# mcogoni/supersdr

Measured on AMD Instinct MI355X. Metric: real-time IQ channels sustained (WF+demod), higher is better.
Workload: dtype f32

## Files before the change

supersdr_amd/csrc/ssdr_audio_dev.h:

```cpp
#pragma once
#include "ssdr_math.h"
#include "ssdr_kernels.h"

constexpr int OCT = 10;
constexpr int NOCT = (SSDR_HIST + SSDR_FRAME) / 8;
constexpr int HOCT = SSDR_HIST / 8;
typedef uint32_t u32x4 __attribute__((ext_vector_type(4)));

SSDR_DEV void lds_sync()
{
    __builtin_amdgcn_fence(__ATOMIC_RELEASE, "wavefront");
    __builtin_amdgcn_wave_barrier();
    __builtin_amdgcn_fence(__ATOMIC_ACQUIRE, "wavefront");
}

template <int CTRL, int ROWMASK>
SSDR_DEV float dpp(float identity, float x)
{
    return __int_as_float(__builtin_amdgcn_update_dpp(__float_as_int(identity), __float_as_int(x), CTRL, ROWMASK, 0xF, false));
}
SSDR_DEV float vmax(float a, float b)
{
    float r;
    asm("v_max_f32 %0, %1, %2" : "=v"(r) : "v"(a), "v"(b));
    return r;
}
SSDR_DEV float vmax3(float a, float b, float c)
{
    float r;
    asm("v_max3_f32 %0, %1, %2, %3" : "=v"(r) : "v"(a), "v"(b), "v"(c));
    return r;
}
SSDR_DEV float vmax3_abs(float a, float b, float c)
{
    float r;
    asm("v_max3_f32 %0, %1, |%2|, |%3|" : "=v"(r) : "v"(a), "v"(b), "v"(c));
    return r;
}
SSDR_DEV uint32_t lane63_u(uint32_t x) { return (uint32_t)__builtin_amdgcn_readlane((int)x, 63); }
SSDR_DEV uint32_t from_prev_lane_u(uint32_t lane0_value, uint32_t x)
{
    return (uint32_t)__builtin_amdgcn_update_dpp((int)lane0_value, (int)x, 0x138, 0xF, 0xF, false);
}
typedef short s16x2 __attribute__((ext_vector_type(2)));
SSDR_DEV uint32_t iq_power(uint32_t raw)
{
    uint32_t p;
    asm("v_dot2_i32_i16 %0, %1, %1, 0" : "=v"(p) : "v"(raw));
    return p;
}
SSDR_DEV float lane63(float x) { return __int_as_float(__builtin_amdgcn_readlane(__float_as_int(x), 63)); }
SSDR_DEV float from_prev_lane(float lane0_value, float x) { return dpp<0x138, 0xF>(lane0_value, x); }

#define SSDR_SCAN6(STEP) STEP("row_shr:1", "0xf") STEP("row_shr:2", "0xf") STEP("row_shr:4", "0xf") STEP("row_shr:8", "0xf") \
                         STEP("row_bcast:15", "0xa") STEP("row_bcast:31", "0xc")
#define SSDR_DPP(C, M) " " C " row_mask:" M " bank_mask:0xf"

SSDR_DEV float scan_max(float x)
{
#define STEP(C, M) asm("s_nop 1\n\tv_max_f32_dpp %0, %0, %0" SSDR_DPP(C, M) : "+v"(x));
    SSDR_SCAN6(STEP)
#undef STEP
    return x;
}
SSDR_DEV float scan_sum(float x)
{
#define STEP(C, M) asm("s_nop 1\n\tv_add_f32_dpp %0, %0, %0" SSDR_DPP(C, M) : "+v"(x));
    SSDR_SCAN6(STEP)
#undef STEP
    return x;
}
SSDR_DEV void scan_affine(float &A, float &B)
{
#define STEP(C, M) asm("s_nop 1\n\tv_fmac_f32_dpp %1, %1, %0" SSDR_DPP(C, M) "\n\tv_mul_f32_dpp %0, %0, %0" SSDR_DPP(C, M) : "+v"(A), "+v"(B));
    SSDR_SCAN6(STEP)
#undef STEP
}

struct Nco {
    uint32_t dphi;
    float cs, ss;
    float qc, qs;
    float tc, ts;
};
SSDR_DEV void nco_setup(Nco &n, uint32_t dphi, int l, int block = 8)
{
    n.dphi = dphi;
    ssdr_phasor32(dphi, n.cs, n.ss);
    ssdr_phasor32((uint32_t)(block * l) * dphi, n.qc, n.qs);
    n.tc = 1.0f; n.ts = 0.0f;
}
SSDR_DEV void nco_frame_table(Nco &n, uint32_t phase_of_frame, int l, int frame = SSDR_FRAME)
{
    ssdr_phasor32(phase_of_frame + (uint32_t)(frame * l) * n.dphi, n.tc, n.ts);
}
SSDR_DEV float lane_f(float x, uint32_t lane) { return __int_as_float(__builtin_amdgcn_readlane(__float_as_int(x), (int)lane)); }
SSDR_DEV void nco_block(const Nco &n, uint32_t f, float &c, float &s)
{
    const float fc = lane_f(n.tc, f & 63u), fs = lane_f(n.ts, f & 63u);
    c = fmaf(fc, n.qc, -(fs * n.qs));
    s = fmaf(fs, n.qc, fc * n.qs);
}
SSDR_DEV void phasor_mul(float ac, float as, float bc, float bs, float &c, float &s)
{
    c = fmaf(ac, bc, -(as * bs));
    s = fmaf(as, bc, ac * bs);
}

template <bool CLIP, int N = 8>
SSDR_DEV void mix8(const uint32_t (&rw)[N], float c, float s, float cs, float ss, float2 (&z)[N], float &amax)
{
#pragma unroll
    for (int j = 0; j < N; j++) {
        const float xr = (float)(int16_t)(rw[j] & 0xFFFFu);
        const float xi = (float)((int32_t)rw[j] >> 16);
        if (CLIP) amax = vmax3_abs(amax, xr, xi);
        z[j] = make_float2(fmaf(xr, c, xi * s), fmaf(xi, c, -(xr * s)));
        const float cn = fmaf(c, cs, -(s * ss)), sn = fmaf(s, cs, c * ss);
        c = cn; s = sn;
    }
}

template <bool CLIP>
SSDR_DEV void mix8_carry(const uint32_t *rw, float &c, float &s, float cs, float ss, float2 (&z)[8], float &amax)
{
#pragma unroll
    for (int j = 0; j < 8; j++) {
        const float xr = (float)(int16_t)(rw[j] & 0xFFFFu);
        const float xi = (float)((int32_t)rw[j] >> 16);
        if (CLIP) amax = vmax3_abs(amax, xr, xi);
        z[j] = make_float2(fmaf(xr, c, xi * s), fmaf(xi, c, -(xr * s)));
        const float cn = fmaf(c, cs, -(s * ss)), sn = fmaf(s, cs, c * ss);
        c = cn; s = sn;
    }
}

SSDR_DEV void load_oct(const float2 *z, int q, float2 (&v)[8])
{
    const float4 *p = reinterpret_cast<const float4 *>(z + q * OCT);
#pragma unroll
    for (int i = 0; i < 4; i++) {
        const float4 t = p[i];
        v[2 * i] = make_float2(t.x, t.y);
        v[2 * i + 1] = make_float2(t.z, t.w);
    }
}

SSDR_DEV void store_oct(float2 *z, int q, const float2 (&v)[8])
{
    float4 *p = reinterpret_cast<float4 *>(z + q * OCT);
#pragma unroll
    for (int i = 0; i < 4; i++) p[i] = make_float4(v[2 * i].x, v[2 * i].y, v[2 * i + 1].x, v[2 * i + 1].y);
}

template <int K0, int NK>
SSDR_DEV void fir_taps(const float *h, const float2 (&A)[8], const float2 (&B)[8], float (&yr)[8], float (&yi)[8])
{
#pragma unroll
    for (int kk = K0; kk < K0 + NK; kk++) {
#pragma unroll
        for (int j = 0; j < 8; j++) {
            const float2 v = (j - kk >= 0) ? A[(j - kk) & 7] : B[(8 + j - kk) & 7];
            yr[j] = fmaf(h[kk], v.x, yr[j]);
            yi[j] = fmaf(h[kk], v.y, yi[j]);
        }
    }
}


struct AgcK { float c0, c1, knee, d8; uint32_t K; };

template <bool INTEGER_POWER>
SSDR_DEV void demod_am(const float (&p)[8], float &dc, float (&aud)[8])
{
    constexpr float DC_APOW[8] = SSDR_DC_APOW_INIT;
    float env[8], loc[8];
    float s = 0.0f;
#pragma unroll
    for (int j = 0; j < 8; j++) {
        env[j] = INTEGER_POWER ? ssdr_sqrt_rn_int(p[j]) : ssdr_sqrt_rn(p[j]);
        s = fmaf(SSDR_DC_A, s, SSDR_DC_AL * env[j]);
        loc[j] = s;
    }
    float Asc = DC_APOW[7], Bsc = s;
    scan_affine(Asc, Bsc);
    const float Ae = from_prev_lane(1.0f, Asc), Be = from_prev_lane(0.0f, Bsc);
    const float carry = fmaf(Ae, dc, Be);
    float m = 0.0f;
#pragma unroll
    for (int j = 0; j < 8; j++) {
        m = fmaf(DC_APOW[j], carry, loc[j]);
        aud[j] = env[j] - m;
    }
    dc = lane63(m);
}

SSDR_DEV void demod_ssb(const float (&yr)[8], const float (&yi)[8], float c, float s, float cs2, float ss2, float (&aud)[8])
{
#pragma unroll
    for (int j = 0; j < 8; j++) {
        aud[j] = fmaf(yr[j], c, -(yi[j] * s));
        const float cn = fmaf(c, cs2, -(s * ss2)), sn = fmaf(s, cs2, c * ss2);
        c = cn; s = sn;
    }
}

SSDR_DEV void demod_fm(const float (&yr)[8], const float (&yi)[8], float prev_re, float prev_im, float kfm, float (&aud)[8])
{
    float pr = from_prev_lane(prev_re, yr[7]), pi = from_prev_lane(prev_im, yi[7]);
#pragma unroll
    for (int j = 0; j < 8; j++) {
        const float dr = fmaf(yr[j], pr, yi[j] * pi);
        const float di = fmaf(yi[j], pr, -(yr[j] * pi));
        aud[j] = ssdr_atan2p(di, dr) * kfm;
        pr = yr[j]; pi = yi[j];
    }
}

SSDR_DEV float block_peak(const float (&p)[8])
{
    return vmax3(vmax3(vmax3(p[0], p[1], p[2]), p[3], p[4]), vmax3(p[5], p[6], p[7]), SSDR_P_FLOOR);
}

SSDR_DEV float agc_pack_store(const float (&p)[8], const float (&aud)[8], int l, const AgcK &k, float &agc_d,
                              float (&agc_m)[8], int16_t *dst, float pm_known = -1.0f)
{
    const float pm = pm_known >= 0.0f ? pm_known : block_peak(p);
    const float al = ssdr_log2p(pm);
    const float fl = (float)l;
    const float d8 = k.d8;
    float e;
    if (k.K == 0) {
        const float P = scan_max(fmaf(fl, d8, al));
        e = vmax(fmaf(-fl, d8, P), fmaf(-(fl + 1.0f), d8, agc_d));
        agc_d = lane63(e);
    } else {
        const float P = scan_max(al);
        float maxM = agc_m[0], mK = agc_m[0];
#pragma unroll
        for (int i = 1; i < 8; i++)
            if ((uint32_t)i < k.K) { maxM = fmaxf(maxM, agc_m[i]); mK = agc_m[i]; }
        e = vmax(vmax(P, maxM), fmaf(-(fl + 1.0f), d8, agc_d));
        agc_d = fmaxf(fmaf(-64.0f, d8, agc_d), mK);
#pragma unroll
        for (int i = 7; i > 0; i--) agc_m[i] = agc_m[i - 1];
        agc_m[0] = lane63(P);
    }
    const float g = ssdr_exp2p(fmaf(k.c1, vmax(e, k.knee), k.c0));
    u32x4 w;
#pragma unroll
    for (int j = 0; j < 8; j += 2) {
        const int i0 = __float2int_rn(aud[j] * g), i1 = __float2int_rn(aud[j + 1] * g);
        w[j >> 1] = __builtin_bit_cast(uint32_t, __builtin_amdgcn_cvt_pk_i16(i0, i1));
    }
    SSDR_NT_STORE(w, reinterpret_cast<u32x4 *>(dst));
    return g;
}

SSDR_DEV void iq_pack_store(const float (&yr)[8], const float (&yi)[8], float g, uint32_t *dst)
{
    u32x4 w0, w1;
#pragma unroll
    for (int j = 0; j < 8; j++) {
        const uint32_t v = __builtin_bit_cast(uint32_t, __builtin_amdgcn_cvt_pk_i16(__float2int_rn(yr[j] * g), __float2int_rn(yi[j] * g)));
        if (j < 4) w0[j] = v; else w1[j - 4] = v;
    }
    SSDR_NT_STORE(w0, reinterpret_cast<u32x4 *>(dst));
    SSDR_NT_STORE(w1, reinterpret_cast<u32x4 *>(dst) + 1);
}

SSDR_DEV void rssi_flag_step(const float (&p)[8], bool clip, uint32_t f, uint32_t n_frames, int l, float cal,
                             float &rssi_sum, uint32_t &flag_keep, float *rssi_row, uint8_t *flag_row)
{
    float ps = p[0];
#pragma unroll
    for (int j = 1; j < 8; j++) ps = ps + p[j];
    const float tot = lane63(scan_sum(ps));
    if ((f & 63u) == (uint32_t)l) { rssi_sum = tot; flag_keep = clip ? 1u : 0u; }
    if ((f & 63u) == 63u || f + 1 == n_frames) {
        if ((uint32_t)l <= (f & 63u)) {
            rssi_row[(f & ~63u) + l] = fmaf(ssdr_log2p(fmaxf(rssi_sum, 1e-20f)) - 39.0f, SSDR_DB_PER_LOG2, cal);
            flag_row[(f & ~63u) + l] = (uint8_t)flag_keep;
        }
    }
}

SSDR_DEV bool wave_any(bool x) { return __builtin_amdgcn_ballot_w64(x) != 0ull; }

SSDR_DEV bool raw_clipped(const uint32_t (&rw)[8])
{
    bool c = false;
#pragma unroll
    for (int j = 0; j < 8; j++) {
        const int lo = (int16_t)(rw[j] & 0xFFFFu), hi = (int32_t)rw[j] >> 16;
        c = c || lo >= 32767 || lo <= -32767 || hi >= 32767 || hi <= -32767;
    }
    return c;
}
```

supersdr_amd/csrc/ssdr_wf.hip:

```cpp
#include "ssdr_math.h"
#include "ssdr_kernels.h"
#include "ssdr_audio_dev.h"
#include "ssdr_wf_dev.h"

namespace {

constexpr int WAVES = SSDR_WF_BLOCK / 64;
constexpr int LDS_TOTAL = LDS_XCH + WAVES * 2 * XCH_FLOATS * 4;
static_assert(LDS_TOTAL <= 163840, "LDS budget");

template <bool AVG, bool HOP>
__global__ __launch_bounds__(SSDR_WF_BLOCK, SSDR_WF_WAVES_PER_EU) void ssdr_wf_kernel(SsdrWfArgs a)
{
    __shared__ __attribute__((aligned(16))) unsigned char smem[LDS_TOTAL];
    load_tables(smem, a.win, a.tw_stage, a.lut);

    const int lane = threadIdx.x & 63, wave = __builtin_amdgcn_readfirstlane(threadIdx.x >> 6);
    const int h = lane >> 5, l = lane & 31;
    float *xch_wave = reinterpret_cast<float *>(smem + LDS_XCH) + wave * 2 * XCH_FLOATS;
    const unsigned char *lut = smem + LDS_LUT0;
    const uint32_t n_pairs = (a.n_ch + 1) >> 1;
    const uint32_t run = HOP ? a.grp_run : 1u;
    const uint32_t n_runs = (a.n_groups + run - 1) / run;
    const uint32_t n_items = n_pairs * n_runs;
    const uint32_t wave_stride = gridDim.x * WAVES;

    for (uint32_t item = blockIdx.x * WAVES + wave; item < n_items; item += wave_stride) {
      uint32_t pair, g_begin, g_end;
      if (HOP) {
          pair = item / n_runs;
          g_begin = (item - pair * n_runs) * run;
          g_end = min(g_begin + run, a.n_groups);
      } else {
          g_begin = item / n_pairs;
          pair = item - g_begin * n_pairs;
          g_end = g_begin + 1;
      }
      const uint32_t n_trips = HOP ? g_end - g_begin : 1u;
      for (uint32_t trip = 0; trip < n_trips; trip++) {
        const uint32_t grp = g_begin + trip;
        uint32_t pair_now = __builtin_amdgcn_readfirstlane(pair);
        asm volatile("" : "+s"(pair_now));
        const WfItem it = wf_item(a, pair_now, grp, h);
        const float calq = a.consts[it.ch].wf_cal_lin * SSDR_LUT_SCALE;
        uint32_t acc[AVG ? 16 : 1];
#pragma unroll
        for (int j = 0; j < (AVG ? 16 : 1); j++) acc[j] = 0;
        constexpr uint32_t LINE_STEP = HOP ? SSDR_NFFT / 2 : SSDR_NFFT;
        const uint32_t *src = a.iq + (uint64_t)it.ch * a.ch_stride + (uint64_t)it.l0 * LINE_STEP + l;

        for (uint32_t line = it.l0; line < it.l1; line++, src += LINE_STEP) {
            f32x2 z[32];
            uint32_t raw[32];
            if (HOP) load_line_halves(line ? src - SSDR_NFFT / 2 : a.tail + (uint64_t)it.ch * (SSDR_NFFT / 2) + l, src, raw);
            else load_line(src, raw);
            if (SSDR_PRIO_WF) prio_compute_phase();
            window_line(raw, smem, l, z);
            SCHED_FENCE();
            fft_line<AVG>(z, smem, xch_wave, h, l);
            if (SSDR_PRIO_WF) prio_latency_phase();

            if (AVG) {
                quantise32(z, calq, lut, [&](int j, uint32_t q01) { acc[j] += q01; });
            } else {
                uint32_t q[16];
                quantise32(z, calq, lut, [&](int j, uint32_t q01) { q[j] = q01; });
                int16_t *x16 = reinterpret_cast<int16_t *>(xch_wave + opaque(h) * XCH_FLOATS) + opaque(l);
#pragma unroll
                for (int j = 0; j < 16; j++) {
                    x16[32 * (j + 16)] = (int16_t)(q[j] & 0xFFFFu);
                    x16[32 * j] = (int16_t)(q[j] >> 16);
                }
            }
        }

        float *xch = xch_wave + opaque(h) * XCH_FLOATS;
        if (AVG) {
            int16_t *x16 = reinterpret_cast<int16_t *>(xch) + opaque(l);
#pragma unroll
            for (int j = 0; j < 16; j++) {
                x16[32 * (j + 16)] = (int16_t)(acc[j] & 0xFFFFu);
                x16[32 * j] = (int16_t)(acc[j] >> 16);
            }
        }
        wave_lds_sync();
        const u32x4 *x128 = reinterpret_cast<const u32x4 *>(xch);
        int16_t *dst = it.complete ? a.out + ((uint64_t)it.grp * a.n_ch + it.ch) * SSDR_NFFT
                                   : a.acc_out + (uint64_t)it.ch * SSDR_NFFT;
        const int16_t *cin = a.acc_in + (uint64_t)it.ch * SSDR_NFFT;
#pragma unroll
        for (int q = 0; q < 4; q++) {
            u32x4 v = x128[q * 32 + l];
            if (AVG && it.carry_in)
                v += reinterpret_cast<const u32x4 *>(cin)[q * 32 + l];
            if (it.ch_ok) SSDR_NT_STORE(v, reinterpret_cast<u32x4 *>(dst) + q * 32 + l);
        }
        wave_lds_sync();
      }
    }
}

template <bool HOP, bool AVG = false>
__global__ __launch_bounds__(SSDR_WF_BLOCK, SSDR_WF_WAVES_PER_EU) void ssdr_fused_am_kernel(SsdrFusedArgs fa)
{
    __shared__ __attribute__((aligned(16))) unsigned char smem[LDS_TOTAL];
    const SsdrWfArgs &a = fa.wf;
    const SsdrAudioArgs &u = fa.au;
    load_tables(smem, a.win, a.tw_stage, a.lut);

    const int lane = threadIdx.x & 63, wave = __builtin_amdgcn_readfirstlane(threadIdx.x >> 6);
    const int h = lane >> 5, l = lane & 31;
    float *xch_wave = reinterpret_cast<float *>(smem + LDS_XCH) + wave * 2 * XCH_FLOATS;
    uint32_t *qbuf = reinterpret_cast<uint32_t *>(xch_wave);
    const unsigned char *lut = smem + LDS_LUT0;
    const uint32_t n_pairs = (a.n_ch + 1) >> 1;
    const uint32_t wave_stride = gridDim.x * WAVES;
    const uint32_t n_frames = u.n_frames;

    for (uint32_t pair = blockIdx.x * WAVES + wave; pair < n_pairs; pair += wave_stride) {
        const uint32_t ch_raw = 2 * pair + h;
        const bool ch_ok = ch_raw < a.n_ch;
        const uint32_t ch = ch_ok ? ch_raw : a.n_ch - 1;
        const float cal_wf = a.consts[ch].wf_cal_lin * SSDR_LUT_SCALE;
        const uint32_t n_sub = (2 * pair + 1 < a.n_ch) ? 2u : 1u;

        float rssi_sum[2] = {0.0f, 0.0f};
        uint32_t flag_keep[2] = {0u, 0u};
        auto pad = [&](int c, int i) -> float & { return xch_wave[c * XCH_FLOATS + 33 * (i + 16) + 32]; };
        if (lane < 2) {
            const uint32_t cc = min(2 * pair + (uint32_t)lane, a.n_ch - 1);
            const ssdr_chan_state st = u.state[cc];
            pad(lane, 0) = st.dc;
            pad(lane, 1) = st.agc_d;
#pragma unroll
            for (int i = 0; i < 8; i++) pad(lane, 2 + i) = st.agc_m[i];
            const uint4 t = *reinterpret_cast<const uint4 *>(u.hist + (size_t)cc * SSDR_HIST + SSDR_HIST - 4);
            pad(lane, 10) = __uint_as_float(iq_power(t.x)); pad(lane, 11) = __uint_as_float(iq_power(t.y));
            pad(lane, 12) = __uint_as_float(iq_power(t.z)); pad(lane, 13) = __uint_as_float(iq_power(t.w));
        }
        wave_lds_sync();

        const uint32_t *src = a.iq + (uint64_t)ch * a.ch_stride + l;
        uint32_t last_raw31 = 0;
        uint32_t acc[AVG ? 16 : 1];
#pragma unroll
        for (int j = 0; j < (AVG ? 16 : 1); j++) acc[j] = 0;
        constexpr uint32_t LINE_STEP = HOP ? SSDR_NFFT / 2 : SSDR_NFFT;
        constexpr int FRAMES_PER_LINE = HOP ? 1 : 2;
        for (uint32_t line = 0; line < a.n_lines; line++, src += LINE_STEP) {
            float dc[2], agc_d[2], agc_m[2][8];
            uint32_t tail_q[2][4];
#pragma unroll
            for (int c = 0; c < 2; c++) {
                dc[c] = pad(c, 0); agc_d[c] = pad(c, 1);
#pragma unroll
                for (int i = 0; i < 8; i++) agc_m[c][i] = pad(c, 2 + i);
#pragma unroll
                for (int i = 0; i < 4; i++) tail_q[c][i] = __float_as_uint(pad(c, 10 + i));
            }
            wave_lds_sync();
            {
                const uint32_t lw = opaque(lane);
                u32x4 t[2][4];
#pragma unroll
                for (int c = 0; c < 2; c++) {
                    uint32_t pair_now = __builtin_amdgcn_readfirstlane(pair);
                    asm volatile("" : "+s"(pair_now));
                    const uint32_t cc = min(2 * pair_now + (uint32_t)c, a.n_ch - 1);
                    const uint32_t *row = a.iq + (uint64_t)cc * a.ch_stride + (uint64_t)line * LINE_STEP;
                    if (HOP) {
                        const uint32_t *older = line ? row - SSDR_NFFT / 2 : a.tail + (uint64_t)cc * (SSDR_NFFT / 2);
#pragma unroll
                        for (int i = 0; i < 2; i++) t[c][i] = SSDR_NT_LOAD(reinterpret_cast<const u32x4 *>(older) + 64 * i + lw);
#pragma unroll
                        for (int i = 0; i < 2; i++) t[c][2 + i] = reinterpret_cast<const u32x4 *>(row)[64 * i + lw];
                    } else {
#pragma unroll
                        for (int i = 0; i < 4; i++) t[c][i] = SSDR_NT_LOAD(reinterpret_cast<const u32x4 *>(row) + 64 * i + lw);
                    }
                }
                SCHED_FENCE();
#pragma unroll
                for (int c = 0; c < 2; c++)
#pragma unroll
                    for (int i = 0; i < 4; i++) reinterpret_cast<u32x4 *>(qbuf + c * XCH_FLOATS)[64 * i + lw] = t[c][i];
                SCHED_FENCE();
            }
            wave_lds_sync();
            prio_latency_phase();
#pragma unroll
            for (int c = 0; c < 2; c++) {
                if ((uint32_t)c >= n_sub) continue;
                uint32_t pair_now = __builtin_amdgcn_readfirstlane(pair);
                asm volatile("" : "+s"(pair_now));
                const uint32_t cc = 2 * pair_now + c;
                const ssdr_chan_consts &kc = u.consts[cc];
                const AgcK agc_c = {kc.agc_c0, kc.agc_c1, kc.agc_knee, kc.agc_delta8, kc.hang_frames};
                const float cal_c = kc.smeter_cal_db;
#pragma unroll
                for (int f = 0; f < FRAMES_PER_LINE; f++) {
                    const uint32_t frame = HOP ? line : 2 * line + f;
                    const u32x4 *qp = reinterpret_cast<const u32x4 *>(qbuf + c * XCH_FLOATS + SSDR_FRAME * (HOP ? 1 : f)) + 2 * opaque(lane);
                    const u32x4 q0 = qp[0], q1 = qp[1];
                    const uint32_t rw[8] = {q0.x, q0.y, q0.z, q0.w, q1.x, q1.y, q1.z, q1.w};
                    uint32_t qv[8], d[8];
#pragma unroll
                    for (int j = 0; j < 8; j++) qv[j] = iq_power(rw[j]);
                    float p[8], aud[8];
#pragma unroll
                    for (int j = 0; j < 4; j++) { d[j] = from_prev_lane_u(tail_q[c][j], qv[4 + j]); d[4 + j] = qv[j]; }
#pragma unroll
                    for (int j = 0; j < 4; j++) tail_q[c][j] = lane63_u(qv[4 + j]);
#pragma unroll
                    for (int j = 0; j < 8; j++) p[j] = (float)d[j];
                    const float pmx = block_peak(p);
                    const bool trig = wave_any(pmx >= 1073676160.0f) || tail_q[c][0] >= 0x3FFF0001u || tail_q[c][1] >= 0x3FFF0001u ||
                                      tail_q[c][2] >= 0x3FFF0001u || tail_q[c][3] >= 0x3FFF0001u;
                    const bool clip = trig ? wave_any(raw_clipped(rw)) : false;
                    demod_am<true>(p, dc[c], aud);
                    agc_pack_store(p, aud, lane, agc_c, agc_d[c], agc_m[c], u.pcm + ((uint64_t)cc * n_frames + frame) * SSDR_FRAME + 8 * lane, pmx);
                    rssi_flag_step(p, clip, frame, n_frames, lane, cal_c, rssi_sum[c], flag_keep[c],
                                   u.rssi + (uint64_t)cc * n_frames, u.flags + (uint64_t)cc * n_frames);
                }
            }
            wave_lds_sync();
            prio_compute_phase();
            uint32_t raw[32];
            {
                const uint32_t *q = qbuf + opaque(h) * XCH_FLOATS + opaque(l);
#pragma unroll
                for (int r = 0; r < 32; r++) raw[r] = q[32 * r];
            }
            wave_lds_sync();
            if (lane < 2) {
#pragma unroll
                for (int c = 0; c < 2; c++) {
                    if (lane != c) continue;
                    pad(c, 0) = dc[c]; pad(c, 1) = agc_d[c];
#pragma unroll
                    for (int i = 0; i < 8; i++) pad(c, 2 + i) = agc_m[c][i];
#pragma unroll
                    for (int i = 0; i < 4; i++) pad(c, 10 + i) = __uint_as_float(tail_q[c][i]);
                }
            }
            wave_lds_sync();
            SCHED_FENCE();
            if (line + 1 == a.n_lines && ch_ok) {
#pragma unroll
                for (int r = 28; r < 32; r++) u.hist[(size_t)ch * SSDR_HIST + 32 * (r - 28) + l] = raw[r];
            }
            last_raw31 = raw[31];
            uint32_t qn[16];
            f32x2 z[32];
            window_line(raw, smem, l, z);
            SCHED_FENCE();
            fft_line<true>(z, smem, xch_wave, h, l);
            prio_latency_phase();
            if (AVG) quantise32(z, cal_wf, lut, [&](int j, uint32_t q01) { acc[j] += q01; });
            else quantise32(z, cal_wf, lut, [&](int j, uint32_t q01) { qn[j] = q01; });
            const uint32_t pos = a.phase + line;
            const bool group_done = !AVG || (pos + 1) % a.n_avg == 0;
            const bool last_line = line + 1 == a.n_lines;
            if (group_done || last_line) {
                float *xch = xch_wave + opaque(h) * XCH_FLOATS;
                int16_t *x16 = reinterpret_cast<int16_t *>(xch) + opaque(l);
#pragma unroll
                for (int j = 0; j < 16; j++) {
                    const uint32_t v = AVG ? acc[j] : qn[j];
                    x16[32 * (j + 16)] = (int16_t)(v & 0xFFFFu);
                    x16[32 * j] = (int16_t)(v >> 16);
                }
                wave_lds_sync();
                const u32x4 *x128 = reinterpret_cast<const u32x4 *>(xch);
                const uint32_t grp = AVG ? pos / a.n_avg : line;
                int16_t *dst = group_done ? a.out + ((uint64_t)grp * a.n_ch + ch) * SSDR_NFFT : a.acc_out + (uint64_t)ch * SSDR_NFFT;
                const bool carry_in = AVG && grp == 0 && a.phase != 0;
                const int16_t *cin = a.acc_in + (uint64_t)ch * SSDR_NFFT;
#pragma unroll
                for (int q = 0; q < 4; q++) {
                    u32x4 v = x128[q * 32 + l];
                    if (carry_in) v += reinterpret_cast<const u32x4 *>(cin)[q * 32 + l];
                    if (ch_ok) SSDR_NT_STORE(v, reinterpret_cast<u32x4 *>(dst) + q * 32 + l);
                }
                wave_lds_sync();
                if (AVG) {
#pragma unroll
                    for (int j = 0; j < 16; j++) acc[j] = 0;
                }
            }
        }

        if (a.n_lines) {
#pragma unroll
            for (int c = 0; c < 2; c++) {
                if ((uint32_t)c >= n_sub) continue;
                const uint32_t cc = 2 * pair + c;
                const ssdr_chan_consts &kc = u.consts[cc];
                ssdr_chan_state st = u.state[cc];
                const uint32_t phi_last = st.phi1 + (uint32_t)(SSDR_FRAME * (n_frames - 1)) * kc.dphi1;
                float fc, fs, qc, qs, bc, bs, cs, ss;
                ssdr_phasor32(phi_last, fc, fs);
                ssdr_phasor32((uint32_t)(8 * 63) * kc.dphi1, qc, qs);
                ssdr_phasor32(kc.dphi1, cs, ss);
                phasor_mul(fc, fs, qc, qs, bc, bs);
#pragma unroll
                for (int j = 0; j < 3; j++) { const float cn = fmaf(bc, cs, -(bs * ss)), sn = fmaf(bs, cs, bc * ss); bc = cn; bs = sn; }
                const float xr = (float)(int16_t)(last_raw31 & 0xFFFFu), xi = (float)((int32_t)last_raw31 >> 16);
                const float zr = fmaf(xr, bc, xi * bs) + 0.0f, zi = fmaf(xi, bc, -(xr * bs)) + 0.0f;
                st.prev_re = lane_f(zr, 32 * c + 27);
                st.prev_im = lane_f(zi, 32 * c + 27);
                st.phi1 += (uint32_t)(SSDR_FRAME * n_frames) * kc.dphi1;
                st.phi2 += (uint32_t)(SSDR_FRAME * n_frames) * kc.dphi2;
                st.dc = pad(c, 0); st.agc_d = pad(c, 1);
#pragma unroll
                for (int i = 0; i < 8; i++) st.agc_m[i] = pad(c, 2 + i);
                if (lane == 0) u.state[cc] = st;
            }
        }
    }
}

__global__ __launch_bounds__(256) void ssdr_quant_selftest_kernel(const float *thr_g, const uint32_t *lut_g,
                                                                    unsigned long long *mismatch)
{
    __shared__ __attribute__((aligned(16))) unsigned char smem[LDS_LUT_END + 16 + 1024];
    float *s_thr = reinterpret_cast<float *>(smem + ((LDS_LUT_END + 15) & ~15));
    uint32_t *s_lut = reinterpret_cast<uint32_t *>(smem + LDS_LUT0);
    for (int i = threadIdx.x; i < 256; i += blockDim.x) s_thr[i] = thr_g[i];
    for (int i = threadIdx.x; i < SSDR_LUT_N; i += blockDim.x) s_lut[i] = lut_g[i];
    __syncthreads();
    unsigned long long bad = 0;
    const unsigned char *lut = smem + LDS_LUT0;
    const uint64_t stride = (uint64_t)gridDim.x * blockDim.x;
    for (uint64_t u = (uint64_t)blockIdx.x * blockDim.x + threadIdx.x; u < 0x7F800000ull; u += stride) {
        const float p = __uint_as_float((uint32_t)u);
        int lo = 0, hi = 255;
        while (lo < hi) {
            const int mid = (lo + hi + 1) >> 1;
            if (s_thr[mid] <= p) lo = mid; else hi = mid - 1;
        }
        float pc;
        asm("v_mul_f32_e64 %0, %1, %2 clamp" : "=v"(pc) : "v"(p), "v"(SSDR_LUT_SCALE));
        bad += (quantise(pc, lut) != (uint32_t)lo);
    }
    if (bad) atomicAdd(mismatch, bad);
}

}

hipError_t ssdr_launch_wf(const SsdrWfArgs &a, uint32_t grid, hipStream_t stream)
{
    const dim3 g(grid), b(SSDR_WF_BLOCK);
    if (a.tail) {
        if (a.n_avg > 1) hipLaunchKernelGGL((ssdr_wf_kernel<true, true>), g, b, 0, stream, a);
        else hipLaunchKernelGGL((ssdr_wf_kernel<false, true>), g, b, 0, stream, a);
    } else {
        if (a.n_avg > 1) hipLaunchKernelGGL((ssdr_wf_kernel<true, false>), g, b, 0, stream, a);
        else hipLaunchKernelGGL((ssdr_wf_kernel<false, false>), g, b, 0, stream, a);
    }
    return hipGetLastError();
}

hipError_t ssdr_launch_fused_am(const SsdrFusedArgs &a, uint32_t grid, hipStream_t stream)
{
    if (a.wf.n_avg > 1) {
        if (a.wf.tail) hipLaunchKernelGGL((ssdr_fused_am_kernel<true, true>), dim3(grid), dim3(SSDR_WF_BLOCK), 0, stream, a);
        else hipLaunchKernelGGL((ssdr_fused_am_kernel<false, true>), dim3(grid), dim3(SSDR_WF_BLOCK), 0, stream, a);
    } else {
        if (a.wf.tail) hipLaunchKernelGGL((ssdr_fused_am_kernel<true, false>), dim3(grid), dim3(SSDR_WF_BLOCK), 0, stream, a);
        else hipLaunchKernelGGL((ssdr_fused_am_kernel<false, false>), dim3(grid), dim3(SSDR_WF_BLOCK), 0, stream, a);
    }
    return hipGetLastError();
}

hipError_t ssdr_fused_blocks_per_cu(int *blocks)
{
    int b[4] = {0, 0, 0, 0};
    hipError_t e = hipOccupancyMaxActiveBlocksPerMultiprocessor(&b[0], ssdr_fused_am_kernel<false, false>, SSDR_WF_BLOCK, 0);
    if (e == hipSuccess) e = hipOccupancyMaxActiveBlocksPerMultiprocessor(&b[1], ssdr_fused_am_kernel<true, false>, SSDR_WF_BLOCK, 0);
    if (e == hipSuccess) e = hipOccupancyMaxActiveBlocksPerMultiprocessor(&b[2], ssdr_fused_am_kernel<false, true>, SSDR_WF_BLOCK, 0);
    if (e == hipSuccess) e = hipOccupancyMaxActiveBlocksPerMultiprocessor(&b[3], ssdr_fused_am_kernel<true, true>, SSDR_WF_BLOCK, 0);
    *blocks = b[0];
    for (int i = 1; i < 4; i++) *blocks = b[i] < *blocks ? b[i] : *blocks;
    return e;
}

hipError_t ssdr_wf_blocks_per_cu(int *blocks)
{
    int b[4] = {0, 0, 0, 0};
    hipError_t e = hipOccupancyMaxActiveBlocksPerMultiprocessor(&b[0], ssdr_wf_kernel<false, false>, SSDR_WF_BLOCK, 0);
    if (e == hipSuccess) e = hipOccupancyMaxActiveBlocksPerMultiprocessor(&b[1], ssdr_wf_kernel<true, false>, SSDR_WF_BLOCK, 0);
    if (e == hipSuccess) e = hipOccupancyMaxActiveBlocksPerMultiprocessor(&b[2], ssdr_wf_kernel<false, true>, SSDR_WF_BLOCK, 0);
    if (e == hipSuccess) e = hipOccupancyMaxActiveBlocksPerMultiprocessor(&b[3], ssdr_wf_kernel<true, true>, SSDR_WF_BLOCK, 0);
    if (e != hipSuccess) return e;
    *blocks = b[0];
    for (int i = 1; i < 4; i++) *blocks = b[i] < *blocks ? b[i] : *blocks;
    return hipSuccess;
}

hipError_t ssdr_launch_quant_selftest(const float *thr, const uint32_t *lut, unsigned long long *mismatch, hipStream_t stream)
{
    hipLaunchKernelGGL(ssdr_quant_selftest_kernel, dim3(2048), dim3(256), 0, stream, thr, lut, mismatch);
    return hipGetLastError();
}
```

Before: 44.15 million.

## Restructure fused AM demod state handling and specialise AGC hang path

Per-channel demod state (dc, AGC, tail powers) moves from the FFT exchange pad into a dedicated per-wave LDS slot. It is now loaded and stored per channel inside the loop instead of being held in registers for both channels across the whole line, which removes one wave sync per line. The DC affine scan hoists its constant multiplier prefix out of the per-frame loop. The AGC path is specialised at compile time on whether a hang ring is used, and the tail carry uses a lane rotate instead of a readlane. The aims are lower register pressure, fewer syncs and less per-frame arithmetic, at the cost of a little extra LDS and larger code.

```diff
diff --git a/supersdr_amd/csrc/ssdr_audio_dev.h b/supersdr_amd/csrc/ssdr_audio_dev.h
--- a/supersdr_amd/csrc/ssdr_audio_dev.h
+++ b/supersdr_amd/csrc/ssdr_audio_dev.h
@@ -42,6 +42,10 @@
 {
     return (uint32_t)__builtin_amdgcn_update_dpp((int)lane0_value, (int)x, 0x138, 0xF, 0xF, false);
 }
+SSDR_DEV uint32_t rot_prev_lane_u(uint32_t x)
+{
+    return (uint32_t)__builtin_amdgcn_mov_dpp((int)x, 0x13C, 0xF, 0xF, false);
+}
 typedef short s16x2 __attribute__((ext_vector_type(2)));
 SSDR_DEV uint32_t iq_power(uint32_t raw)
 {
@@ -73,6 +77,26 @@
 SSDR_DEV void scan_affine(float &A, float &B)
 {
 #define STEP(C, M) asm("s_nop 1\n\tv_fmac_f32_dpp %1, %1, %0" SSDR_DPP(C, M) "\n\tv_mul_f32_dpp %0, %0, %0" SSDR_DPP(C, M) : "+v"(A), "+v"(B));
+    SSDR_SCAN6(STEP)
+#undef STEP
+}
+struct DcScan {
+    float a[6];
+    float ae;
+};
+SSDR_DEV void dc_scan_setup(DcScan &d, float a0)
+{
+    float A = a0;
+    int k = 0;
+#define STEP(C, M) d.a[k++] = A; asm("s_nop 1\n\tv_mul_f32_dpp %0, %0, %0" SSDR_DPP(C, M) : "+v"(A));
+    SSDR_SCAN6(STEP)
+#undef STEP
+    d.ae = dpp<0x138, 0xF>(1.0f, A);
+}
+SSDR_DEV void scan_affine_b(const DcScan &d, float &B)
+{
+    int k = 0;
+#define STEP(C, M) asm("s_nop 1\n\tv_fmac_f32_dpp %0, %0, %1" SSDR_DPP(C, M) : "+v"(B) : "v"(d.a[k])); k++;
     SSDR_SCAN6(STEP)
 #undef STEP
 }
@@ -194,6 +218,29 @@
     }
     dc = lane63(m);
 }
+SSDR_DEV void demod_am_int(const float (&p)[8], const DcScan &ds, float &dc, float (&aud)[8])
+{
+    constexpr float DC_APOW[8] = SSDR_DC_APOW_INIT;
+    float env[8], loc[8];
+    float s = 0.0f;
+#pragma unroll
+    for (int j = 0; j < 8; j++) {
+        env[j] = ssdr_sqrt_rn_int(p[j]);
+        s = fmaf(SSDR_DC_A, s, SSDR_DC_AL * env[j]);
+        loc[j] = s;
+    }
+    float Bsc = s;
+    scan_affine_b(ds, Bsc);
+    const float Be = from_prev_lane(0.0f, Bsc);
+    const float carry = fmaf(ds.ae, dc, Be);
+    float m = 0.0f;
+#pragma unroll
+    for (int j = 0; j < 8; j++) {
+        m = fmaf(DC_APOW[j], carry, loc[j]);
+        aud[j] = env[j] - m;
+    }
+    dc = lane63(m);
+}
 
 SSDR_DEV void demod_ssb(const float (&yr)[8], const float (&yi)[8], float c, float s, float cs2, float ss2, float (&aud)[8])
 {
@@ -222,15 +269,16 @@
     return vmax3(vmax3(vmax3(p[0], p[1], p[2]), p[3], p[4]), vmax3(p[5], p[6], p[7]), SSDR_P_FLOOR);
 }
 
+template <int HANG = 0>
 SSDR_DEV float agc_pack_store(const float (&p)[8], const float (&aud)[8], int l, const AgcK &k, float &agc_d,
                               float (&agc_m)[8], int16_t *dst, float pm_known = -1.0f)
 {
-    const float pm = pm_known >= 0.0f ? pm_known : block_peak(p);
+    const float pm = HANG || pm_known >= 0.0f ? pm_known : block_peak(p);
     const float al = ssdr_log2p(pm);
     const float fl = (float)l;
     const float d8 = k.d8;
     float e;
-    if (k.K == 0) {
+    if (HANG == 1 || (HANG == 0 && k.K == 0)) {
         const float P = scan_max(fmaf(fl, d8, al));
         e = vmax(fmaf(-fl, d8, P), fmaf(-(fl + 1.0f), d8, agc_d));
         agc_d = lane63(e);
diff --git a/supersdr_amd/csrc/ssdr_wf.hip b/supersdr_amd/csrc/ssdr_wf.hip
--- a/supersdr_amd/csrc/ssdr_wf.hip
+++ b/supersdr_amd/csrc/ssdr_wf.hip
@@ -8,6 +8,9 @@
 constexpr int WAVES = SSDR_WF_BLOCK / 64;
 constexpr int LDS_TOTAL = LDS_XCH + WAVES * 2 * XCH_FLOATS * 4;
 static_assert(LDS_TOTAL <= 163840, "LDS budget");
+constexpr int LDS_FUSED_ST = LDS_TOTAL;
+constexpr int LDS_FUSED = LDS_FUSED_ST + WAVES * 32 * 4;
+static_assert(LDS_FUSED_ST % 16 == 0 && LDS_FUSED <= 163840 / 2, "two workgroups per CU");
 
 template <bool AVG, bool HOP>
 __global__ __launch_bounds__(SSDR_WF_BLOCK, SSDR_WF_WAVES_PER_EU) void ssdr_wf_kernel(SsdrWfArgs a)
@@ -103,7 +106,7 @@
 template <bool HOP, bool AVG = false>
 __global__ __launch_bounds__(SSDR_WF_BLOCK, SSDR_WF_WAVES_PER_EU) void ssdr_fused_am_kernel(SsdrFusedArgs fa)
 {
-    __shared__ __attribute__((aligned(16))) unsigned char smem[LDS_TOTAL];
+    __shared__ __attribute__((aligned(16))) unsigned char smem[LDS_FUSED];
     const SsdrWfArgs &a = fa.wf;
     const SsdrAudioArgs &u = fa.au;
     load_tables(smem, a.win, a.tw_stage, a.lut);
@@ -112,6 +115,7 @@
     const int h = lane >> 5, l = lane & 31;
     float *xch_wave = reinterpret_cast<float *>(smem + LDS_XCH) + wave * 2 * XCH_FLOATS;
     uint32_t *qbuf = reinterpret_cast<uint32_t *>(xch_wave);
+    float *st_wave = reinterpret_cast<float *>(smem + LDS_FUSED_ST) + wave * 32;
     const unsigned char *lut = smem + LDS_LUT0;
     const uint32_t n_pairs = (a.n_ch + 1) >> 1;
     const uint32_t wave_stride = gridDim.x * WAVES;
@@ -126,19 +130,18 @@
 
         float rssi_sum[2] = {0.0f, 0.0f};
         uint32_t flag_keep[2] = {0u, 0u};
-        auto pad = [&](int c, int i) -> float & { return xch_wave[c * XCH_FLOATS + 33 * (i + 16) + 32]; };
         if (lane < 2) {
             const uint32_t cc = min(2 * pair + (uint32_t)lane, a.n_ch - 1);
             const ssdr_chan_state st = u.state[cc];
-            pad(lane, 0) = st.dc;
-            pad(lane, 1) = st.agc_d;
-#pragma unroll
-            for (int i = 0; i < 8; i++) pad(lane, 2 + i) = st.agc_m[i];
+            float *s = st_wave + 16 * lane;
+            s[0] = st.dc;
+            s[1] = st.agc_d;
+#pragma unroll
+            for (int i = 0; i < 8; i++) s[8 + i] = st.agc_m[i];
             const uint4 t = *reinterpret_cast<const uint4 *>(u.hist + (size_t)cc * SSDR_HIST + SSDR_HIST - 4);
-            pad(lane, 10) = __uint_as_float(iq_power(t.x)); pad(lane, 11) = __uint_as_float(iq_power(t.y));
-            pad(lane, 12) = __uint_as_float(iq_power(t.z)); pad(lane, 13) = __uint_as_float(iq_power(t.w));
-        }
-        wave_lds_sync();
+            s[4] = __uint_as_float(iq_power(t.x)); s[5] = __uint_as_float(iq_power(t.y));
+            s[6] = __uint_as_float(iq_power(t.z)); s[7] = __uint_as_float(iq_power(t.w));
+        }
 
         const uint32_t *src = a.iq + (uint64_t)ch * a.ch_stride + l;
         uint32_t last_raw31 = 0;
@@ -148,16 +151,6 @@
         constexpr uint32_t LINE_STEP = HOP ? SSDR_NFFT / 2 : SSDR_NFFT;
         constexpr int FRAMES_PER_LINE = HOP ? 1 : 2;
         for (uint32_t line = 0; line < a.n_lines; line++, src += LINE_STEP) {
-            float dc[2], agc_d[2], agc_m[2][8];
-            uint32_t tail_q[2][4];
-#pragma unroll
-            for (int c = 0; c < 2; c++) {
-                dc[c] = pad(c, 0); agc_d[c] = pad(c, 1);
-#pragma unroll
-                for (int i = 0; i < 8; i++) agc_m[c][i] = pad(c, 2 + i);
-#pragma unroll
-                for (int i = 0; i < 4; i++) tail_q[c][i] = __float_as_uint(pad(c, 10 + i));
-            }
             wave_lds_sync();
             {
                 const uint32_t lw = opaque(lane);
@@ -188,6 +181,11 @@
             }
             wave_lds_sync();
             prio_latency_phase();
+            DcScan dcs;
+            {
+                constexpr float DC_APOW[8] = SSDR_DC_APOW_INIT;
+                dc_scan_setup(dcs, DC_APOW[7]);
+            }
 #pragma unroll
             for (int c = 0; c < 2; c++) {
                 if ((uint32_t)c >= n_sub) continue;
@@ -197,30 +195,57 @@
                 const ssdr_chan_consts &kc = u.consts[cc];
                 const AgcK agc_c = {kc.agc_c0, kc.agc_c1, kc.agc_knee, kc.agc_delta8, kc.hang_frames};
                 const float cal_c = kc.smeter_cal_db;
-#pragma unroll
-                for (int f = 0; f < FRAMES_PER_LINE; f++) {
-                    const uint32_t frame = HOP ? line : 2 * line + f;
-                    const u32x4 *qp = reinterpret_cast<const u32x4 *>(qbuf + c * XCH_FLOATS + SSDR_FRAME * (HOP ? 1 : f)) + 2 * opaque(lane);
-                    const u32x4 q0 = qp[0], q1 = qp[1];
-                    const uint32_t rw[8] = {q0.x, q0.y, q0.z, q0.w, q1.x, q1.y, q1.z, q1.w};
-                    uint32_t qv[8], d[8];
-#pragma unroll
-                    for (int j = 0; j < 8; j++) qv[j] = iq_power(rw[j]);
-                    float p[8], aud[8];
-#pragma unroll
-                    for (int j = 0; j < 4; j++) { d[j] = from_prev_lane_u(tail_q[c][j], qv[4 + j]); d[4 + j] = qv[j]; }
-#pragma unroll
-                    for (int j = 0; j < 4; j++) tail_q[c][j] = lane63_u(qv[4 + j]);
-#pragma unroll
-                    for (int j = 0; j < 8; j++) p[j] = (float)d[j];
-                    const float pmx = block_peak(p);
-                    const bool trig = wave_any(pmx >= 1073676160.0f) || tail_q[c][0] >= 0x3FFF0001u || tail_q[c][1] >= 0x3FFF0001u ||
-                                      tail_q[c][2] >= 0x3FFF0001u || tail_q[c][3] >= 0x3FFF0001u;
-                    const bool clip = trig ? wave_any(raw_clipped(rw)) : false;
-                    demod_am<true>(p, dc[c], aud);
-                    agc_pack_store(p, aud, lane, agc_c, agc_d[c], agc_m[c], u.pcm + ((uint64_t)cc * n_frames + frame) * SSDR_FRAME + 8 * lane, pmx);
-                    rssi_flag_step(p, clip, frame, n_frames, lane, cal_c, rssi_sum[c], flag_keep[c],
-                                   u.rssi + (uint64_t)cc * n_frames, u.flags + (uint64_t)cc * n_frames);
+                float *s = st_wave + 16 * c;
+                float dc = s[0], agc_d = s[1];
+                uint32_t tail_v[4];
+#pragma unroll
+                for (int i = 0; i < 4; i++) tail_v[i] = __float_as_uint(s[4 + i]);
+                auto frames = [&](auto hang, float (&agc_m)[8]) {
+#pragma unroll
+                    for (int f = 0; f < FRAMES_PER_LINE; f++) {
+                        const uint32_t frame = HOP ? line : 2 * line + f;
+                        const u32x4 *qp = reinterpret_cast<const u32x4 *>(qbuf + c * XCH_FLOATS + SSDR_FRAME * (HOP ? 1 : f)) + 2 * opaque(lane);
+                        const u32x4 q0 = qp[0], q1 = qp[1];
+                        const uint32_t rw[8] = {q0.x, q0.y, q0.z, q0.w, q1.x, q1.y, q1.z, q1.w};
+                        uint32_t qv[8], d[8];
+#pragma unroll
+                        for (int j = 0; j < 8; j++) qv[j] = iq_power(rw[j]);
+                        float p[8], aud[8];
+#pragma unroll
+                        for (int j = 0; j < 4; j++) {
+                            d[j] = from_prev_lane_u(tail_v[j], qv[4 + j]); d[4 + j] = qv[j];
+                            tail_v[j] = rot_prev_lane_u(qv[4 + j]);
+                        }
+#pragma unroll
+                        for (int j = 0; j < 8; j++) p[j] = (float)d[j];
+                        const float pmx = block_peak(p);
+                        const uint32_t tmx = max(max(tail_v[0], tail_v[1]), max(tail_v[2], tail_v[3]));
+                        const bool trig = wave_any(pmx >= 1073676160.0f || tmx >= 0x3FFF0001u);
+                        const bool clip = trig ? wave_any(raw_clipped(rw)) : false;
+                        demod_am_int(p, dcs, dc, aud);
+                        agc_pack_store<decltype(hang)::value>(p, aud, lane, agc_c, agc_d, agc_m,
+                                                              u.pcm + ((uint64_t)cc * n_frames + frame) * SSDR_FRAME + 8 * lane, pmx);
+                        rssi_flag_step(p, clip, frame, n_frames, lane, cal_c, rssi_sum[c], flag_keep[c],
+                                       u.rssi + (uint64_t)cc * n_frames, u.flags + (uint64_t)cc * n_frames);
+                    }
+                };
+                if (agc_c.K == 0) {
+                    float no_ring[8];
+                    frames(std::integral_constant<int, 1>(), no_ring);
+                } else {
+                    float agc_m[8];
+#pragma unroll
+                    for (int i = 0; i < 8; i++) agc_m[i] = s[8 + i];
+                    frames(std::integral_constant<int, 2>(), agc_m);
+                    if (lane == 0) {
+#pragma unroll
+                        for (int i = 0; i < 8; i++) s[8 + i] = agc_m[i];
+                    }
+                }
+                if (lane == 0) {
+                    s[0] = dc; s[1] = agc_d;
+#pragma unroll
+                    for (int i = 0; i < 4; i++) s[4 + i] = __uint_as_float(tail_v[i]);
                 }
             }
             wave_lds_sync();
@@ -230,18 +255,6 @@
                 const uint32_t *q = qbuf + opaque(h) * XCH_FLOATS + opaque(l);
 #pragma unroll
                 for (int r = 0; r < 32; r++) raw[r] = q[32 * r];
-            }
-            wave_lds_sync();
-            if (lane < 2) {
-#pragma unroll
-                for (int c = 0; c < 2; c++) {
-                    if (lane != c) continue;
-                    pad(c, 0) = dc[c]; pad(c, 1) = agc_d[c];
-#pragma unroll
-                    for (int i = 0; i < 8; i++) pad(c, 2 + i) = agc_m[c][i];
-#pragma unroll
-                    for (int i = 0; i < 4; i++) pad(c, 10 + i) = __uint_as_float(tail_q[c][i]);
-                }
             }
             wave_lds_sync();
             SCHED_FENCE();
@@ -311,9 +324,9 @@
                 st.prev_im = lane_f(zi, 32 * c + 27);
                 st.phi1 += (uint32_t)(SSDR_FRAME * n_frames) * kc.dphi1;
                 st.phi2 += (uint32_t)(SSDR_FRAME * n_frames) * kc.dphi2;
-                st.dc = pad(c, 0); st.agc_d = pad(c, 1);
-#pragma unroll
-                for (int i = 0; i < 8; i++) st.agc_m[i] = pad(c, 2 + i);
+                st.dc = st_wave[16 * c]; st.agc_d = st_wave[16 * c + 1];
+#pragma unroll
+                for (int i = 0; i < 8; i++) st.agc_m[i] = st_wave[16 * c + 8 + i];
                 if (lane == 0) u.state[cc] = st;
             }
         }
```

Measured after the change: 44.63 million, median of 6. 1.01x the previous value.
